# taindp98/Endoscopy-Image-Classification

Measured on AMD Instinct MI355X. Metric: unlabeled images/sec/node (FixMatch ViT-S, 224², μ=7), higher is better.
Workload: dtype bf16; 1 GPU; F1: FixMatch ViT-S/16 step, global B=64 labeled + mu*B=448 unlabeled weak/strong pairs (64 + 448 per GPU, strong scaling), 224^2, C=23, tau=0.95, lambda_u=1, Adam 1e-3, EMA 0.999; global_batch=960, seq_len=197, parallelism=dp1, hipgraph=False

## Files before the change

endoscopy-image-classification_amd/csrc/gemm.hip:

```cpp
#include <algorithm>
#include <mutex>
#include <type_traits>

#include <hip/hip_ext.h>

#include "common.h"

namespace es_gemm {

constexpr int BM = 128, BN = 128, BK = 64;

enum Epi {
  EPI_BF16 = 0,
  EPI_GELU = 1,
  EPI_F32_RESID = 2,
  EPI_DGELU = 3,
  EPI_F32 = 4,
  EPI_PATCH = 5,
  EPI_GELU_ACT = 6,
  EPI_GELU_D = 7,
  EPI_MULAUX = 8,
};

struct NTArgs {
// ... 1403 lines not shown
          const float2 rr = rv[2 * s + q / (RPS / 2)][q % (RPS / 2)][j];
          v[j] = make_float2(t.x + rr.x, t.y + rr.y);
        }
        if constexpr (s == 0)
          if (q == RPS / 2 - 1) load_resid(std::integral_constant<int, 3>{});
        const LnRow384 o = ln_row384(v, (q & 1) == 0, l.eps, gam_lds, bet_lds, lane);
        const int m = m0 + tile_row(s, q);
        const bool ok = m < p.M;
#pragma unroll
        for (int j = 0; j < 3; ++j) {
          const int c = (j * 64 + lane) * 2;
          __builtin_amdgcn_raw_buffer_store_b64(__builtin_bit_cast(u32x2, v[j]), rx,
                                                ok ? (unsigned)(m * p.ldc + c) * 4u : ES_OOB, 0, 0);
          __builtin_amdgcn_raw_buffer_store_b32(o.h[j], rh, ok ? (unsigned)(m * l.ldh + c) * 2u : ES_OOB, 0, 0);
        }
        const bool one = ok && lane == 0;
        __builtin_amdgcn_raw_buffer_store_b32(__builtin_bit_cast(unsigned, o.mean), rm,
                                              one ? (unsigned)m * 4u : ES_OOB, 0, 0);
        __builtin_amdgcn_raw_buffer_store_b32(__builtin_bit_cast(unsigned, o.rstd), rs,
                                              one ? (unsigned)m * 4u : ES_OOB, 0, 0);
      }
    };
    slab(std::integral_constant<int, 0>{});
    asm volatile("s_waitcnt lgkmcnt(0)" ::: "memory");
    __builtin_amdgcn_s_barrier();
    slab(std::integral_constant<int, 1>{});
    if (tid == 0) qslot[0] = claimed;
    asm volatile("s_waitcnt lgkmcnt(0)" ::: "memory");
    __builtin_amdgcn_s_barrier();
    cur = __builtin_amdgcn_readfirstlane(qslot[0]);
  }
  TILE_CTR_RELEASE(ctr, tid)
}
#undef TILE_CTR_RELEASE

#define NT_LAUNCH(E, BKT_, NST_, TBM_, ...)                                             \
  {                                                                                        \
    const size_t lds = std::max((size_t)NST_ * (TBM_ + BN) * BKT_ * 2, (size_t)4 * EPI_WAVE_BYTES); \
    allow_lds(gemm_nt_kernel<E, BKT_, NST_, TBM_, ##__VA_ARGS__>, lds);                   \
    hipLaunchKernelGGL(HIP_KERNEL_NAME(gemm_nt_kernel<E, BKT_, NST_, TBM_, ##__VA_ARGS__>), dim3(grid), dim3(256), lds, stream, a); \
    return ES_OK;                                                                          \
  }
#define NT_EPIS(BKT_, NST_, TBM_, ...)                                            \
  switch (epi) {                                                                  \
    case EPI_BF16: NT_LAUNCH(EPI_BF16, BKT_, NST_, TBM_, ##__VA_ARGS__)           \
    case EPI_GELU: NT_LAUNCH(EPI_GELU, BKT_, NST_, TBM_, ##__VA_ARGS__)           \
    case EPI_F32_RESID: NT_LAUNCH(EPI_F32_RESID, BKT_, NST_, TBM_, ##__VA_ARGS__) \
    case EPI_DGELU: NT_LAUNCH(EPI_DGELU, BKT_, NST_, TBM_, ##__VA_ARGS__)         \
    case EPI_F32: NT_LAUNCH(EPI_F32, BKT_, NST_, TBM_, ##__VA_ARGS__)             \
    case EPI_PATCH: NT_LAUNCH(EPI_PATCH, BKT_, NST_, TBM_, ##__VA_ARGS__)         \
    case EPI_GELU_ACT: NT_LAUNCH(EPI_GELU_ACT, BKT_, NST_, TBM_, ##__VA_ARGS__)   \
    case EPI_GELU_D: NT_LAUNCH(EPI_GELU_D, BKT_, NST_, TBM_, ##__VA_ARGS__)       \
    case EPI_MULAUX: NT_LAUNCH(EPI_MULAUX, BKT_, NST_, TBM_, ##__VA_ARGS__)       \
    default: return ES_BAD_ARG;                                                   \
  }
int launch_nt(int cfg, int epi, int grid, hipStream_t stream, const NTArgs& a) {
  if (cfg == 11 && epi == EPI_F32_RESID) NT_LAUNCH(EPI_F32_RESID, 64, 2, 64, 0)
  switch (cfg) {
    case 0: NT_EPIS(64, 2, 128)
    case 5: NT_EPIS(32, 2, 128)
    case 11: NT_EPIS(64, 2, 64)
    default: NT_EPIS(32, 3, 128)
  }
}
#undef NT_EPIS
#undef NT_LAUNCH
// ... 41 lines not shown
  if (n < CTR_SLOTS) {
    tab[n] = s;
    return n++;
  }
  return (int)(((uintptr_t)s >> 6) % CTR_SLOTS);
}
static int persistent_grid(int tiles) {
  static const int cus = [] {
    int dev = 0, n = 0;
    (void)hipGetDevice(&dev);
    return (hipDeviceGetAttribute(&n, hipDeviceAttributeMultiprocessorCount, dev) != hipSuccess || n <= 0) ? 256 : n;
  }();
  return std::max(1, std::min(cus, tiles));
}

int launch_resid_ln(hipStream_t stream, const NTArgs& a, const RLArgs& l) {
  const int grid = persistent_grid((a.M + rlg::R - 1) / rlg::R);
  allow_lds(gemm_resid_ln_kernel, (size_t)rlg::LDS);
  hipLaunchKernelGGL(gemm_resid_ln_kernel, dim3(grid), dim3(512), rlg::LDS, stream, a, l, tile_ctr_slot(stream));
  return hipGetLastError() == hipSuccess ? ES_OK : ES_HIP_ERROR;
}

int launch_nt_ln(int ring, hipStream_t stream, const NTArgs& a, const RLArgs& l) {
  const int grid = persistent_grid((a.M + nlg::TBM - 1) / nlg::TBM);
  const int slot = tile_ctr_slot(stream);
  constexpr size_t lds3 = nlg::lds<3, 32>(), lds2 = nlg::lds<2, 64>();
  if (ring == 1) {
    allow_lds(gemm_nt_ln_kernel<3, 32>, lds3);
    hipLaunchKernelGGL(HIP_KERNEL_NAME(gemm_nt_ln_kernel<3, 32>), dim3(grid), dim3(512), lds3, stream, a, l, slot);
  } else {
    allow_lds(gemm_nt_ln_kernel<2, 64>, lds2);
    hipLaunchKernelGGL(HIP_KERNEL_NAME(gemm_nt_ln_kernel<2, 64>), dim3(grid), dim3(512), lds2, stream, a, l, slot);
  }
  return hipGetLastError() == hipSuccess ? ES_OK : ES_HIP_ERROR;
}

}
using namespace es_gemm;

static int g_gemm_variant = -1;
static int g_tn_variant = -1;
static int g_small_tile = 1;

extern "C" {

int es_gemm_tn_ex(const void* A1, int ld1, const void* A2, int ld2, int M, int N1, int N2, int splits,
                  float* workspace, float* out, int accumulate, float* bias_out, int variant, hipStream_t stream);

int es_gemm_nt(int epi, const void* A, int lda, const void* B, int ldb, const float* bias, void* C,
               int ldc, void* C2, const void* aux, int ldaux, int M, int N, int K, int np,
               hipStream_t stream) {
  if (M <= 0 || N <= 0 || K <= 0 || (N % BN) || (K % BK) || (lda % 8) || (ldb % 8) || (ldc % 4))
    return ES_BAD_SHAPE;
  if (!A || !B || !C) return ES_BAD_ARG;
  if (((epi == EPI_GELU || epi == EPI_GELU_D) && !C2) ||
      ((epi == EPI_F32_RESID || epi == EPI_DGELU || epi == EPI_MULAUX || epi == EPI_PATCH) && !aux))
    return ES_BAD_ARG;
  if (epi == EPI_PATCH && np <= 0) return ES_BAD_ARG;
  if ((epi == EPI_F32_RESID || epi == EPI_PATCH) && ((ldaux % 4) || ldaux < N)) return ES_BAD_SHAPE;
  if ((epi == EPI_DGELU || epi == EPI_MULAUX) && ((ldaux % 8) || ldaux < N)) return ES_BAD_SHAPE;
  NTArgs a{(const bf16*)A, (const bf16*)B, bias, C, C2, aux, M, N, K, lda, ldb, ldc, ldaux, np};
  int variant = g_gemm_variant;
  if (variant < 0) {
    const bool gelu = epi == EPI_GELU || epi == EPI_GELU_ACT || epi == EPI_GELU_D;
    const bool plain = epi == EPI_BF16 || epi == EPI_F32 || epi == EPI_F32_RESID || epi == EPI_MULAUX;
    if (g_small_tile && N <= 384 && ((K <= 384 && epi == EPI_F32_RESID) || (M < 32768 && (plain || epi == EPI_GELU_ACT))))
// ... 56 lines not shown
      (size_t)M * (size_t)std::max(ldc, ldaux) * 4 >= (1u << 31))
    return ES_BAD_SHAPE;
  if (!A || !B || !C || !aux || !gamma || !beta || !h || !mean || !rstd) return ES_BAD_ARG;
  if ((((uintptr_t)A | (uintptr_t)aux | (uintptr_t)B | (uintptr_t)gamma | (uintptr_t)beta) & 15) ||
      (bias && ((uintptr_t)bias & 15)) || ((uintptr_t)C & 7) || ((uintptr_t)h & 3))
    return ES_BAD_ARG;
  NTArgs a{(const bf16*)A, (const bf16*)B, bias, C, nullptr, aux, M, N, K, lda, ldb, ldc, ldaux, 0};
  RLArgs l{gamma, beta, (bf16*)h, mean, rstd, ldh, eps};
  return launch_resid_ln(stream, a, l);
}

static int g_nt_ln_ring = 0;
int es_gemm_nt_ln(const void* A, int lda, const void* B, int ldb, const float* bias, float* C, int ldc,
                  const float* aux, int ldaux, const float* gamma, const float* beta, void* h, int ldh, float* mean,
                  float* rstd, int M, int N, int K, float eps, hipStream_t stream) {
  if (M <= 0 || N != nlg::D || K <= 0 || (K % 64) || (lda % 8) || (ldb % 8) || (ldc % 2) || (ldaux % 2) || (ldh % 2) ||
      lda < K || ldb < K || ldc < N || ldaux < N || ldh < N ||
      (size_t)M * (size_t)std::max(std::max(ldc, ldaux), ldh) * 4 >= (1u << 31))
    return ES_BAD_SHAPE;
  if (!A || !B || !C || !aux || !gamma || !beta || !h || !mean || !rstd) return ES_BAD_ARG;
  if ((((uintptr_t)A | (uintptr_t)B | (uintptr_t)gamma | (uintptr_t)beta) & 15) || (bias && ((uintptr_t)bias & 15)) ||
      (((uintptr_t)C | (uintptr_t)aux) & 7) || (((uintptr_t)h | (uintptr_t)mean | (uintptr_t)rstd) & 3))
    return ES_BAD_ARG;
  NTArgs a{(const bf16*)A, (const bf16*)B, bias, C, nullptr, aux, M, N, K, lda, ldb, ldc, ldaux, 0};
  RLArgs l{gamma, beta, (bf16*)h, mean, rstd, ldh, eps};
  return launch_nt_ln(g_nt_ln_ring, stream, a, l);
}
int endossl_nt_ln_ring(int v) {
  const int old = g_nt_ln_ring;
  g_nt_ln_ring = v == 1 ? 1 : 0;
  return old;
}

static bool gemm_variant_ok(int v) {
  return v == -1 || v == 0 || v == 1 || v == 2 || v == 5 || v == 6 || v == 10 || v == 11;
}
int es_set_gemm_variant(int v) {
  if (!gemm_variant_ok(v)) return ES_BAD_ARG;
  const int old = g_gemm_variant;
  g_gemm_variant = v;
  return old;
}

int es_set_gemm_small_tile(int v) {
  const int old = g_small_tile;
  g_small_tile = v;
  return old;
}

int es_set_tn_variant(int v) {
  if (v != -1 && v != 0 && v != 7) return ES_BAD_ARG;
  const int old = g_tn_variant;
  g_tn_variant = v;
  return old;
}

constexpr int TN_MIN_SPLIT_TOKENS = 512;
static bool tn_big_ok(int N1, int N2, int ld1, int ld2) {
  return N1 % TB1 == 0 && N2 % TB2 == 0 && ld1 % 8 == 0 && ld2 % 8 == 0;
}
static int tn_pick(int M, int N1, int N2, int ld1, int ld2, int v) {
  if (!(N1 % BM == 0 && N2 % BN == 0)) return 7;
  if (v == 7) return tn_big_ok(N1, N2, ld1, ld2) ? 7 : 0;
  if (v >= 0) return 0;
  return (tn_big_ok(N1, N2, ld1, ld2) && M >= 65536) ? 7 : 0;
}
// ... 259 lines not shown
```

endoscopy-image-classification_amd/endossl/_lib.py:

```python
import ctypes
import os

import torch

_HERE = os.path.dirname(os.path.abspath(__file__))
LIB_PATH = os.environ.get("ENDOSSL_LIB", os.path.join(_HERE, "lib", "libendossl_hip.so"))

V, I, L, F, Z = ctypes.c_void_p, ctypes.c_int, ctypes.c_long, ctypes.c_float, ctypes.c_size_t
U64 = ctypes.c_ulonglong

SIGNATURES = {
    "es_abi_version": (I, []),
    "es_gemm_nt": (I, [I, V, I, V, I, V, V, I, V, V, I, I, I, I, I, V]),
    "es_gemm_nt_resid_ln": (I, [V, I, V, I, V, V, I, V, I, V, V, V, I, V, V, I, I, I, F, V]),
    "es_gemm_nt_ln": (I, [V, I, V, I, V, V, I, V, I, V, V, V, I, V, V, I, I, I, F, V]),
    "es_set_gemm_variant": (I, [I]),
    "es_set_gemm_small_tile": (I, [I]),
    "es_gemm_tn_workspace": (Z, [I, I, I]),
    "es_gemm_tn": (I, [V, I, V, I, I, I, I, I, V, V, I, V, V]),
    "es_gemm_tn_ex": (I, [V, I, V, I, I, I, I, I, V, V, I, V, I, V]),
    "es_set_tn_variant": (I, [I]),
    "es_set_attn_variant": (I, [I]),
    "es_set_attn_bwd_variant": (I, [I]),
    "es_set_attn_bwd_grid": (I, [I]),
    "es_set_ln_fwd_grid": (I, [I]),
    "es_set_attn_bwd_long": (I, [I]),
    "es_splitk_reduce": (I, [V, V, I, I, I, V]),
    "es_tn_problem_size": (Z, []),
    "es_gemm_tn_grouped_prepare": (I, [V, I]),
    "es_gemm_tn_grouped": (I, [V, I, I, V]),
    "es_set_stem_kernels": (I, [I]),
    "es_gemm_tn_big_grouped_table_bytes": (Z, [I]),
    "es_gemm_tn_big_grouped_workspace": (Z, [V, I, I]),
    "es_gemm_tn_big_grouped_prepare": (I, [V, I, I, V, Z, V, V]),
    "es_gemm_tn_big_grouped": (I, [V, I, V, V]),
    "es_gemm_tn_big_grouped_timed": (I, [V, I, V, V, V, V]),
    "es_event_create": (I, [V]),
    "es_event_elapsed": (I, [V, V, V]),
    "es_event_destroy": (I, [V]),
    "es_colsum": (I, [V, I, I, I, V, I, V, I, V]),
    "es_attn_fwd": (I, [V, I, V, I, V, I, I, I, F, V]),
    "es_attn_bwd": (I, [V, I, V, I, V, V, V, I, V, I, I, I, I, F, V]),
    "es_attn_cls_fwd": (I, [V, I, V, I, V, I, I, I, F, V]),
    "es_attn_cls_bwd": (I, [V, I, V, I, V, V, I, V, I, I, I, I, F, V]),
    "es_reduce_partials": (I, [V, V, I, I, I, V]),
    "es_layernorm_fwd": (I, [V, I, V, V, V, I, V, V, I, I, F, V]),
    "es_layernorm_bwd": (I, [V, I, V, I, V, V, V, V, I, V, I, V, I, V, V, V, I, I, I, I, V]),
    "es_layernorm_bwd_b16": (I, [V, I, V, I, V, V, V, V, I, V, I, V, I, V, V, V, I, I, I, I, V]),
    "es_layernorm_bwd_grid": (I, [I, I]),
    "es_ln_param_grads_entry_size": (I, []),
    "es_ln_param_grads_multi": (I, [V, I, V]),
    "es_gelu_fwd": (I, [V, V, L, V]),
    "es_gelu_bwd": (I, [V, V, V, L, V]),
    "es_patch_im2col": (I, [V, V, I, I, I, V]),
    "es_patch_im2col_u8": (I, [V, F, F, F, F, F, F, V, I, I, I, V]),
    "es_cls_init": (I, [V, I, V, V, I, I, I, V]),
    "es_embed_bwd": (I, [V, I, V, I, V, V, I, I, I, I, V]),
    "es_cls_head_fwd": (I, [V, I, I, V, V, V, V, V, I, V, V, I, I, I, F, V]),
    "es_cls_head_bwd": (I, [V, I, V, V, V, V, V, V, V, I, I, V, V, V, V, I, I, I, V]),
    "es_cls_head_bwd_ex": (I, [V, I, V, V, V, V, V, V, V, I, I, V, V, V, V, I, I, I, I, V]),
    "es_cls_ln_fwd": (I, [V, I, I, V, V, V, I, V, V, I, I, F, V]),
    "es_cls_ln_bwd": (I, [V, I, V, V, V, V, I, I, V, V, I, I, V]),
    "es_dense_fwd": (I, [V, I, V, V, V, I, I, I, I, I, F, V, F, V]),
    "es_dense_bwd_workspace": (Z, [I, I]),
    "es_dense_bwd": (I, [V, I, V, I, I, F, V, F, V, I, V, V, I, I, V, V, I, I, I, V, V]),
    "es_bn1d_fwd": (I, [V, I, V, V, V, V, V, F, F, I, V, I, V, V, I, I, V]),
    "es_bn1d_bwd": (I, [V, I, V, V, V, V, I, V, V, I, I, V]),
    "es_dropout_keep": (I, [V, L, F, U64, U64, V]),
    "es_bn1d_sums": (I, [V, I, I, I, V, F, V, V]),
    "es_bn1d_fwd_global": (I, [V, I, V, V, V, V, F, V, V, V, F, F, V, I, V, V, I, I, V]),
    "es_bn1d_bwd_sums": (I, [V, I, V, I, I, V, V]),
    "es_bn1d_bwd_global": (I, [V, I, V, V, V, V, V, F, V, I, V, V, I, I, V]),
    "es_l2norm_fwd": (I, [V, I, V, I, V, I, I, V]),
    "es_l2norm_bwd": (I, [V, I, V, I, V, V, I, I, I, V]),
    "es_comatch_pseudo_workspace": (Z, [I, I, I]),
    "es_comatch_pseudo": (I, [V, I, I, I, V, I, I, I, V, I, I, V, V, I, F, F, F, V, V, V, V, V, V]),
    "es_comatch_pseudo_ex": (I, [V, I, I, I, V, I, I, I, I, V, I, I, V, V, I, F, F, F, V, V, V, V, V, V]),
    "es_softmax_colmean": (I, [V, I, I, I, V, V]),
    "es_comatch_bank_write": (I, [V, I, I, V, I, I, I, V, V, I, V, V, I, I, V]),
    "es_comatch_contrastive_workspace": (Z, [I]),
    "es_comatch_contrastive_fwd_bwd": (I, [V, I, V, I, V, I, I, I, F, F, F, V, V, I, V, I, V, V]),
    "es_comatch_contrastive_ex_workspace": (Z, [I, I]),
    "es_comatch_contrastive_fwd_bwd_ex": (I, [V, I, V, I, V, V, I, I, I, I, I, F, F, F, F, V, V, I, V, I, V, V]),
    "es_comatch_focal_fwd_bwd": (I, [V, I, V, V, I, I, F, F, V, V, I, V, V]),
    "es_fm_consistency_fwd_bwd": (I, [V, I, V, I, I, I, F, F, V, V, V, V, I, V, V]),
    "es_poly_ce_fwd_bwd": (I, [V, I, V, V, I, I, F, F, V, I, V, V]),
    "es_triplet_fwd_bwd": (I, [V, I, I, I, F, F, V, I, V, V]),
    "es_softmax_predict": (I, [V, I, I, I, F, V, V, V, V]),
    "es_margin_softmax_workspace": (Z, [I, I]),
# ... 194 lines not shown
```

endoscopy-image-classification_amd/endossl/vit.py:

```python
import ctypes
import functools
import math
import os

import torch
import torch.nn as nn

from . import _lib, block
from ._lib import call, ptr
from .block import (EPI_BF16, EPI_DGELU, EPI_F32, EPI_F32_RESID, EPI_GELU, EPI_GELU_ACT,
                    EPI_GELU_D, EPI_MULAUX, EPI_PATCH, Rows, _TNProblem)

LN_BWD_BLOCKS = 1024
SIDE_PRIORITY = -1
SIDE_PRIORITY_MIN_M = 65536


IMAGENET_MEAN = (0.485, 0.456, 0.406)
IMAGENET_STD = (0.229, 0.224, 0.225)


def _rup(x, m):
    return (x + m - 1) // m * m

# ... 72 lines not shown
                nn.init.uniform_(t, -bound, bound, generator=generator)
            elif name.startswith(("fc.", "head_emb.")):
                if name == "fc.3.weight":
                    t.fill_(1.0)
                elif name == "fc.3.bias":
                    t.zero_()
                elif len(shape) == 2:
                    nn.init.kaiming_uniform_(t, a=math.sqrt(5), generator=generator)
                else:
                    w = [sh for nm, sh in layout if nm == name[:-len("bias")] + "weight"][0]
                    bound = 1.0 / math.sqrt(w[1])
                    nn.init.uniform_(t, -bound, bound, generator=generator)
            elif name.startswith("head"):
                t.zero_()
            elif name.endswith("weight") and len(shape) == 2:
                nn.init.trunc_normal_(t, std=0.02, generator=generator)
            elif "norm" in name and name.endswith("weight"):
                t.fill_(1.0)
            else:
                t.zero_()


class _Acts:

    def __init__(self, cfg, n, train, device, b16=torch.bfloat16):
        D, Hd, L = cfg.dim, cfg.hidden, cfg.depth
        self.n, self.train = n, train
        self.M = n * cfg.T
        Mp = _rup(self.M, 256) + 256
        self.Mp = Mp
        Lk = L if train else 1
        f32 = torch.float32
        z = lambda *s, dt=f32: torch.zeros(*s, dtype=dt, device=device)
        self.patches = z(_rup(n * cfg.np, 256), 3 * cfg.patch * cfg.patch, dt=b16)
        self.x = z(L + 1 if train else 2, Mp, D)
        self.xmid = z(Lk, Mp, D)
        self.h1 = z(Lk, Mp, D, dt=b16)
        self.h2 = z(Lk, Mp, D, dt=b16)
        self.mean1, self.rstd1 = z(Lk, Mp), z(Lk, Mp)
        self.mean2, self.rstd2 = z(Lk, Mp), z(Lk, Mp)
        self.qkv = z(Lk, Mp, 3 * D, dt=b16)
        self.o = z(Lk, Mp, D, dt=b16)
        self.lse = z(Lk, n * cfg.heads * cfg.T)
        self.pre = z(Lk if train else 0, Mp, Hd, dt=b16)
        self.act = z(Lk, Mp, Hd, dt=b16)
        Mc = _rup(n, 256)
        self.c_o, self.c_lse = z(Mc, D, dt=b16), z(n * cfg.heads)
        self.c_h1 = z(Mc, D, dt=b16)
        self.c_xmid, self.c_h2 = z(Mc, D), z(Mc, D, dt=b16)
        self.c_mean2, self.c_rstd2 = z(Mc), z(Mc)
        self.c_pre = z(Mc, Hd, dt=b16) if train else None
        self.c_act, self.c_xout = z(Mc, Hd, dt=b16), z(Mc, D)
        self.xhat = z(n, D)
        self.rstd_cls = z(n)
        self.logits = z(n, cfg.num_classes)
        self.fts = z(n, D) if cfg.head == "emb" else None


class _Grads:

    def __init__(self, cfg, n, device, b16=torch.bfloat16):
        D, Hd = cfg.dim, cfg.hidden
        Mp = _rup(n * cfg.T, 256) + 256
        f32 = torch.float32
        z = lambda *s, dt=f32: torch.zeros(*s, dtype=dt, device=device)
        self.n = n
        self.dx, self.dxb = z(Mp, D), z(Mp, D, dt=b16)
        self.dxm, self.dxmb = z(Mp, D), z(Mp, D, dt=b16)
        self.dh = z(Mp, D, dt=b16) if Engine.DH_BF16 else z(Mp, D)
        self.dpre = z(Mp, Hd, dt=b16)
        self.dqkv = z(Mp, 3 * D, dt=b16)
        self.do = z(Mp, D, dt=b16)
        self.dpatch = z(_rup(n * cfg.np, 256), D, dt=b16)
        self.dyn = z(n, D)
        self.delta = z(n * cfg.heads * cfg.T)
        Mc = _rup(n, 256)
        self.c_dx, self.c_dxb = z(Mc, D), z(Mc, D, dt=b16)
        self.c_dpre, self.c_dxmb, self.c_do = z(Mc, Hd, dt=b16), z(Mc, D, dt=b16), z(Mc, D, dt=b16)
        self.c_dh = z(Mc, D, dt=b16) if Engine.DH_BF16 else z(Mc, D)
        self.dxm_cls = z(Mp, D)


class _WgradSchedule:

    def __init__(self, sets, M, depth, grouped, *, layer_wgrad, defer_ln, bf16, capture, group_layers, min_m, main,
                 side, wgrad, wgrad_layer, launch_grouped, ln_flush, grad_ready=None, block_range=None,
                 on_stream=block.on_stream):
        self.mode = "grouped" if grouped else "layer" if layer_wgrad and bf16 and M >= min_m else "each"
        self.defer = [] if defer_ln and grad_ready is None and not capture and self.mode != "each" else None
# ... 52 lines not shown
            self._launch_grouped(self.problems, 0)
        if self.defer:
            self._ln_flush(self.defer)
        if self.side is not None:
            self.main.wait_stream(self.side)


class Engine:

    TN_TARGET_BLOCKS = 768
    TN_SHARE = 0.5
    TN_SHARE_MIN_M = 16384
    TN_MAX_SPLITS = 128
    GROUP_WGRAD = "auto"
    GROUP_WGRAD_MAX_M = 16384
    GROUP_LAYERS = 6
    DEFER_LN_GRADS = True
    LN_MULTI_MAX = 32
    LAYER_WGRAD = True
    LAYER_TN_SHARE = 0.375
    _OV = os.environ.get("ENDOSSL_OVERLAP", "1")
    OVERLAP_FWD = _OV in ("1", "fwd")
    OVERLAP = _OV in ("1", "bwd")
    DH_BF16 = True
    GELU_D = True
    PRUNE_LAST = True
    PRUNE_Q = True
    RESID_LN = os.environ.get("ENDOSSL_RESID_LN", "1") == "1"
    RESID_LN_MIN_M = 40000
    FC2_LN = os.environ.get("ENDOSSL_FC2_LN", "1") == "1"
    FC2_LN_MIN_M = 50000
    FC2_LN_TRAIN = True
    FC2_LN_WEAK = True

    PARITY_NAMES = {n: n + "_f32" for n in (
        "es_gemm_nt", "es_gemm_tn", "es_attn_fwd", "es_attn_bwd", "es_attn_cls_fwd", "es_attn_cls_bwd",
        "es_layernorm_fwd", "es_layernorm_bwd", "es_patch_im2col", "es_patch_im2col_u8", "es_embed_bwd",
        "es_pack_weights")}
    PARITY_NAMES.update({"es_layernorm_bwd_b16": "es_layernorm_bwd_f32", "es_cast_f32_bf16": "es_copy_f32"})

    def __init__(self, cfg, device, precision="bf16"):
        if precision not in ("bf16", "fp32"):
            raise ValueError(f"precision must be 'bf16' (production) or 'fp32' (parity mode), got {precision!r}")
        self.cfg, self.device = cfg, device
        self.precision = precision
        self.op_dtype = torch.bfloat16 if precision == "bf16" else torch.float32
        self.layout, self.offs, self.numel = param_layout(cfg)
        self.shapes = dict(self.layout)
        self._acts = {}
        self._grads = {}
        self._ws = None
        self._ws_ln = None
        self._ws_lnp = None
        self._lnp_next = 0
        self._side = None
        self._ncu_cache = None
        self._gtab = {}
        self._grad_b = None
        self.overlap = self.OVERLAP
        self.overlap_fwd = self.OVERLAP_FWD
        self._packed_version = -1
        D, Hd = cfg.dim, cfg.hidden
        b16 = self.op_dtype
        mats = [("patch_embed.proj.weight", D, 3 * cfg.patch * cfg.patch, False)]
        for i in range(cfg.depth):
            b = f"blocks.{i}."
# ... 58 lines not shown
        if self._ws is None:
            cfg = self.cfg
            D, Hd = cfg.dim, cfg.hidden
            n_tn = max(a * b for a, b in ((3 * D, D), (D, D), (Hd, D), (D, Hd), (D, 3 * cfg.patch * cfg.patch)))
            self._ws = torch.empty(self.TN_MAX_SPLITS * n_tn + 2 * 1024 * max(Hd, 3 * D), dtype=torch.float32,
                                   device=self.device)
        return self._ws

    def ln_workspace(self):
        if self._ws_ln is None:
            self._ws_ln = torch.empty(2 * LN_BWD_BLOCKS * self.cfg.dim, dtype=torch.float32, device=self.device)
        return self._ws_ln

    def _ncu(self):
        if self._ncu_cache is None:
            self._ncu_cache = torch.cuda.get_device_properties(self.device).multi_processor_count
        return self._ncu_cache

    def side_stream(self, tokens=0):
        prio = SIDE_PRIORITY if tokens >= SIDE_PRIORITY_MIN_M else 0
        if self._side is None:
            self._side = {}
        if prio not in self._side:
            self._side[prio] = torch.cuda.Stream(device=self.device, priority=prio)
        return self._side[prio]

    def forward(self, flat, images_list, train):
        cfg = self.cfg
        s = _lib.stream()
        n = sum(int(t.shape[0]) for t in images_list)
        A = self.acts(n, train)
        D, T, H = cfg.dim, cfg.T, cfg.heads
        K0 = 3 * cfg.patch * cfg.patch
        row = 0
        for t in images_list:
            if t.shape[1:] != (3, cfg.img_size, cfg.img_size) or t.dtype not in (torch.float32, torch.uint8):
                raise ValueError(f"expected fp32 (normalised) or uint8 (raw) [n,3,{cfg.img_size},{cfg.img_size}] "
                                 f"images, got {tuple(t.shape)} {t.dtype}")
            t = t.contiguous()
            if t.dtype == torch.uint8:
                self._call("es_patch_im2col_u8", ptr(t), *IMAGENET_MEAN, *IMAGENET_STD, ptr(A.patches[row * cfg.np:]),
                     int(t.shape[0]), cfg.img_size, cfg.patch, s)
            else:
                self._call("es_patch_im2col", ptr(t), ptr(A.patches[row * cfg.np:]), int(t.shape[0]), cfg.img_size,
                     cfg.patch, s)
            row += int(t.shape[0])
        x0 = A.x[0]
        pos = self.view(flat, "pos_embed")
        block.gemm_nt(self._call, EPI_PATCH, A.patches, self.wb["patch_embed.proj.weight"],
                      self.view(flat, "patch_embed.proj.bias"), x0, n * cfg.np, D, K0, aux=pos, ldaux=D, npatch=cfg.np)
        self._call("es_cls_init", ptr(x0), D, ptr(self.view(flat, "cls_token")), ptr(pos), n, T, D, s)
        M = A.M
        prune = self._prune()
        ch = self._chain(flat)
        fused = self.RESID_LN and D == 384 and self.precision == "bf16" and M >= self.RESID_LN_MIN_M
        fc2_ln = (self.FC2_LN and (self.FC2_LN_TRAIN if train else self.FC2_LN_WEAK) and D == 384
                  and self.precision == "bf16" and M >= self.FC2_LN_MIN_M)
        ln_done = False
        for i in range(cfg.depth):
            b = f"blocks.{i}."
            li = i if train else 0
            xin = A.x[i] if train else A.x[i & 1]
            xout = A.x[i + 1] if train else A.x[(i + 1) & 1]
            R = Rows(n, T, H, x=xin, h1=A.h1[li], mean1=A.mean1[li], rstd1=A.rstd1[li], qkv=A.qkv[li], o=A.o[li],
                     lse=A.lse[li], xmid=A.xmid[li], h2=A.h2[li], mean2=A.mean2[li], rstd2=A.rstd2[li],
                     pre=A.pre[li] if train else None, act=A.act[li], out=xout)
            if prune and i == cfg.depth - 1:
                Rc = self._cls_rows(A, n, xin)
                ch.attn_fwd(b, R, cls=Rc, split_q=self.PRUNE_Q, ln_done=ln_done)
                ch.mlp_fwd(b, Rc, train)
                if self.capture is not None:
                    self.capture("fwd_cls", train, i, xin[:M], A.c_xout[:n])
                break
            ch.attn_fwd(b, R, ln_done=ln_done)
            next_ln = None
            if fc2_ln and i + 1 < cfg.depth:
                nb, ni = f"blocks.{i + 1}.", i + 1 if train else 0
                next_ln = (self.view(flat, nb + "norm1.weight"), self.view(flat, nb + "norm1.bias"), A.h1[ni],
                           A.mean1[ni], A.rstd1[ni])
            ch.mlp_fwd(b, R, train, fused=fused, label="fc1_fwd" if train else "fc1_fwd_weak", next_ln=next_ln)
            ln_done = next_ln is not None
            if self.capture is not None:
                self.capture("fwd", train, i, xin[:M], xout[:M])
        xl = A.x[cfg.depth] if train else A.x[cfg.depth & 1]
        Tl = T
        if prune:
            xl, Tl = A.c_xout, 1
        if cfg.head == "emb":
            self._call("es_cls_ln_fwd", ptr(xl), D, Tl, ptr(self.view(flat, "norm.weight")),
                 ptr(self.view(flat, "norm.bias")), ptr(A.fts), D, ptr(A.xhat), ptr(A.rstd_cls), n, D, cfg.eps, s)
            return A.fts
# ... 346 lines not shown
```

include/endossl.h:

```cpp
#ifndef ENDOSSL_H
#define ENDOSSL_H
#include <stddef.h>
#include <stdint.h>
#include <hip/hip_runtime_api.h>

#ifdef __cplusplus
extern "C" {
#endif

int es_abi_version(void);

int es_gemm_nt(int epi, const void* A, int lda, const void* B, int ldb, const float* bias, void* C, int ldc,
               void* C2, const void* aux, int ldaux, int M, int N, int K, int np, hipStream_t stream);
int es_gemm_nt_resid_ln(const void* A, int lda, const void* B, int ldb, const float* bias, float* C, int ldc,
                        const float* aux, int ldaux, const float* gamma, const float* beta, void* h, int ldh,
                        float* mean, float* rstd, int M, int N, int K, float eps, hipStream_t stream);
int es_gemm_nt_ln(const void* A, int lda, const void* B, int ldb, const float* bias, float* C, int ldc,
                  const float* aux, int ldaux, const float* gamma, const float* beta, void* h, int ldh, float* mean,
                  float* rstd, int M, int N, int K, float eps, hipStream_t stream);
int es_set_gemm_variant(int variant);
int es_set_gemm_small_tile(int v);
int es_set_tn_variant(int variant);
size_t es_gemm_tn_workspace(int N1, int N2, int splits);
int es_gemm_tn(const void* A1, int ld1, const void* A2, int ld2, int M, int N1, int N2, int splits,
// ... 54 lines not shown
int es_ln_param_grads_entry_size(void);
int es_ln_param_grads_multi(const void* table, int n, hipStream_t stream);

int es_gelu_fwd(const void* x, void* y, long n, hipStream_t stream);
int es_gelu_bwd(const void* x, const void* dy, void* dx, long n, hipStream_t stream);

size_t es_aug_entry_size(void);
size_t es_aug_strong_workspace(int n, int S);
size_t es_aug_fixmatch_workspace(int n, int S, int is_crop, int max_w, int max_h);
int es_aug_fixmatch_u8(const uint8_t* frames, size_t frames_bytes, const void* entries, const int32_t* coeffs,
                       size_t coeff_count, int n, int S, int is_crop, int max_h, uint8_t* weak, uint8_t* strong,
                       void* workspace, size_t workspace_bytes, hipStream_t stream);
int es_aug_strong_u8(const uint8_t* weak, const void* entries, int n, int S, uint8_t* strong, void* workspace,
                     size_t workspace_bytes, hipStream_t stream);

size_t es_aug_comatch_entry_size(void);
size_t es_aug_labeled_entry_size(void);
size_t es_aug_comatch_workspace(int n, int S, int is_crop, int max_w, int max_h);
size_t es_aug_labeled_workspace(int n, int S, int is_crop, int max_w, int max_h);
int es_aug_comatch_u8(const uint8_t* frames, size_t frames_bytes, const void* entries, const int32_t* coeffs,
                      size_t coeff_count, int n, int S, int is_crop, int max_h, uint8_t* weak, uint8_t* strong0,
                      uint8_t* strong1, void* workspace, size_t workspace_bytes, hipStream_t stream);
int es_aug_labeled_u8(const uint8_t* frames, size_t frames_bytes, const void* entries, const int32_t* coeffs,
                      size_t coeff_count, int n, int S, int is_crop, int max_h, uint8_t* out, void* workspace,
                      size_t workspace_bytes, hipStream_t stream);
int es_aug_jitter_u8(const uint8_t* x, const void* plans, int n, int S, uint8_t* out, hipStream_t stream);


int es_patch_im2col(const float* img, void* patches, int n, int S, int P, hipStream_t stream);

int es_patch_im2col_u8(const void* img, float mean0, float mean1, float mean2, float std0, float std1, float std2,
                       void* patches, int n, int S, int P, hipStream_t stream);
int es_cls_init(float* x, int ldx, const float* cls, const float* pos, int n, int T, int D, hipStream_t stream);
int es_embed_bwd(const float* dx, int lddx, void* dpatch, int ldp, float* dpos, float* dcls, int n, int T, int D,
                 int accumulate, hipStream_t stream);
int es_cls_head_fwd(const float* x, int ldx, int T, const float* gamma, const float* beta, const float* W,
                    const float* b, float* logits, int ldl, float* xhat, float* rstd, int n, int D, int C, float eps,
                    hipStream_t stream);
int es_cls_head_bwd(const float* dl, int lddl, const float* W, const float* gamma, const float* beta,
                    const float* xhat, const float* rstd, float* dyn, float* dx, int lddx, int T, float* dW, float* db,
                    float* dgamma, float* dbeta, int n, int D, int C, hipStream_t stream);
int es_cls_head_bwd_ex(const float* dl, int lddl, const float* W, const float* gamma, const float* beta,
                       const float* xhat, const float* rstd, float* dyn, float* dx, int lddx, int T, float* dW,
                       float* db, float* dgamma, float* dbeta, int n, int D, int C, int accumulate, hipStream_t stream);

int es_cls_ln_fwd(const float* x, int ldx, int T, const float* gamma, const float* beta, float* fts, int ldf,
                  float* xhat, float* rstd, int n, int D, float eps, hipStream_t stream);
int es_cls_ln_bwd(const float* dfts, int lddf, const float* gamma, const float* xhat, const float* rstd, float* dx,
                  int lddx, int T, float* dgamma, float* dbeta, int n, int D, hipStream_t stream);

int es_dense_fwd(const float* X, int ldx, const float* W, const float* b, float* Y, int ldy, int n, int K, int N,
                 int act, float slope, const void* keep, float keep_scale, hipStream_t stream);
size_t es_dense_bwd_workspace(int n, int N);
int es_dense_bwd(const float* dY, int lddy, const float* Yact, int ldya, int act, float slope, const void* keep,
                 float keep_scale, const float* X, int ldx, const float* W, float* dX, int lddx, int accumulate_dx,
                 float* dW, float* db, int n, int K, int N, float* workspace, hipStream_t stream);
int es_bn1d_fwd(const float* U, int ldu, const float* gamma, const float* beta, float* running_mean, float* running_var,
                void* num_batches_tracked, float momentum, float eps, int train, float* Y, int ldy, float* xhat,
                float* rstd, int n, int F, hipStream_t stream);
int es_bn1d_bwd(const float* dY, int lddy, const float* xhat, const float* rstd, const float* gamma, float* dU,
                int lddu, float* dgamma, float* dbeta, int n, int F, hipStream_t stream);
int es_bn1d_sums(const float* U, int ldu, int n, int F, const float* S1, float N, float* out, hipStream_t stream);
int es_bn1d_fwd_global(const float* U, int ldu, const float* gamma, const float* beta, const float* S1,
                       const float* S2, float N, float* running_mean, float* running_var, void* num_batches_tracked,
                       float momentum, float eps, float* Y, int ldy, float* xhat, float* rstd, int n, int F,
                       hipStream_t stream);
// ... 267 lines not shown
```

Measured before the change: 15380 unlabeled images/s.

## Fuse uint8 im2col, patch-embed GEMM, pos add and first LayerNorm into one kernel

Adds a persistent patch-embedding kernel that reads raw uint8 images directly, normalises them through an LDS lookup table into the GEMM A tile, adds bias and positional embedding, and computes block 0's norm1 LayerNorm in the epilogue. A companion kernel writes the CLS row plus its LayerNorm, and the patch buffer is allocated lazily and only written when training needs it for the backward pass. This removes the separate im2col pass, one activation round trip and a standalone LayerNorm launch, at the cost of a more complex kernel with per-thread image address computation and gathered A loads instead of async global-to-LDS copies.

```diff
diff --git a/endoscopy-image-classification_amd/csrc/gemm.hip b/endoscopy-image-classification_amd/csrc/gemm.hip
--- a/endoscopy-image-classification_amd/csrc/gemm.hip
+++ b/endoscopy-image-classification_amd/csrc/gemm.hip
@@ -1459,6 +1459,266 @@
   }
   TILE_CTR_RELEASE(ctr, tid)
 }
+
+struct PEArgs {
+  const uint8_t* img[4];
+  int pstart[4];
+  int S, G, np;
+  float mean[3], std[3];
+  bf16* patches;
+};
+namespace peg {
+constexpr int BKT = 64, NST = 2, KD = 768;
+constexpr int BODY = nlg::body<NST, BKT>();
+constexpr int LDS = BODY + 16 + nlg::D * 4 * 3 + 3 * 256 * 2;
+}
+
+__global__ __launch_bounds__(512, 1) void patch_embed_ln_kernel(NTArgs p, RLArgs l, PEArgs e, int slot) {
+  using namespace nlg;
+  constexpr int BKT = peg::BKT;
+  extern __shared__ __attribute__((aligned(16))) char smem[];
+  constexpr int ROWB = BKT * 2, RPI = 1024 / ROWB, CPR = ROWB / 16, RPW = 8 * RPI;
+  constexpr int IB = D / RPW;
+  constexpr int TA = TBM * ROWB, STAGE = (TBM + D) * ROWB;
+  int* const qslot = (int*)(smem + peg::BODY);
+  float* const bias_lds = (float*)(smem + peg::BODY + 16);
+  float* const gam_lds = bias_lds + D;
+  float* const bet_lds = gam_lds + D;
+  unsigned short* const tab = (unsigned short*)(bet_lds + D);
+  const int tid = threadIdx.x, lane = tid & 63;
+  const int w = __builtin_amdgcn_readfirstlane(tid >> 6);
+  const int wm = w / WN, wn = w % WN;
+  const int g = lane >> 4, r = lane & 15;
+  int* const ctr = g_tile_ctr + slot * CTR_INTS;
+  const int nt = (p.M + TBM - 1) / TBM;
+  if (tid == 0) qslot[0] = __hip_atomic_fetch_add(ctr, 1, __ATOMIC_RELAXED, __HIP_MEMORY_SCOPE_AGENT);
+  if (tid < D / 4) {
+    *(f32x4*)(bias_lds + 4 * tid) = p.bias ? *(const f32x4*)(p.bias + 4 * tid) : f32x4{0.f, 0.f, 0.f, 0.f};
+    *(f32x4*)(gam_lds + 4 * tid) = *(const f32x4*)(l.gamma + 4 * tid);
+    *(f32x4*)(bet_lds + 4 * tid) = *(const f32x4*)(l.beta + 4 * tid);
+  }
+  for (int i = tid; i < 3 * 256; i += 512) {
+    const int c = i >> 8;
+    const float mu = c == 0 ? e.mean[0] : (c == 1 ? e.mean[1] : e.mean[2]);
+    const float sd = c == 0 ? e.std[0] : (c == 1 ? e.std[1] : e.std[2]);
+    const bf16 v = (bf16)(((float)(i & 255) / 255.0f - mu) / sd);
+    tab[i] = __builtin_bit_cast(unsigned short, v);
+  }
+  __syncthreads();
+  int cur = __builtin_amdgcn_readfirstlane(qslot[0]);
+
+  const bf16* gb[IB];
+#pragma unroll
+  for (int j = 0; j < IB; ++j) {
+    const int row = (j * 8 + w) * RPI + lane / CPR;
+    gb[j] = p.B + (size_t)row * p.ldb + swzk<BKT>(row, lane % CPR) * 8;
+  }
+  const int pr = tid >> 2, kyi = tid & 3;
+  const unsigned aoff0 = pr * ROWB + (swzk<BKT>(pr, 2 * kyi) << 4), aoff1 = pr * ROWB + (swzk<BKT>(pr, 2 * kyi + 1) << 4);
+  const unsigned T = (unsigned)e.np + 1u, rows = (unsigned)(p.M / e.np) * T;
+  const __amdgpu_buffer_rsrc_t rx = buf_rsrc(p.C, rows * p.ldc * 4u);
+  const __amdgpu_buffer_rsrc_t rh = buf_rsrc(l.h, rows * l.ldh * 2u);
+  const __amdgpu_buffer_rsrc_t rm = buf_rsrc(l.mean, rows * 4u);
+  const __amdgpu_buffer_rsrc_t rs = buf_rsrc(l.rstd, rows * 4u);
+  const __amdgpu_buffer_rsrc_t rp = buf_rsrc(e.patches ? (void*)e.patches : p.C, e.patches ? (unsigned)p.M * peg::KD * 2u : 0u);
+  const float* const pos = (const float*)p.aux;
+  constexpr int nk = peg::KD / BKT;
+  const size_t plane = (size_t)e.S * e.S;
+
+  while (cur < nt) {
+    const int m0 = cur * TBM, last = p.M - 1;
+    auto tile_row = [&](int s, int q) {
+      const int lr = w * RPS + q;
+      return (lr >> 5) * 64 + s * 32 + (lr & 31);
+    };
+    float2 rv[4][RPS / 2][3];
+    auto load_pos = [&](auto gc) {
+      constexpr int gi = decltype(gc)::value;
+#pragma unroll
+      for (int q = 0; q < RPS / 2; ++q) {
+        const int mm = min(m0 + tile_row(gi >> 1, (gi & 1) * (RPS / 2) + q), last);
+        const float* xr = pos + (size_t)(1 + mm % e.np) * p.ldaux;
+#pragma unroll
+        for (int j = 0; j < 3; ++j) rv[gi][q][j] = *(const float2*)(xr + (j * 64 + lane) * 2);
+      }
+    };
+
+    const int am = min(m0 + pr, last);
+    const int ti = (am >= e.pstart[1]) + (am >= e.pstart[2]) + (am >= e.pstart[3]);
+    const uint8_t* const ib = ti == 0 ? e.img[0] : (ti == 1 ? e.img[1] : (ti == 2 ? e.img[2] : e.img[3]));
+    const int lm = am - (ti == 0 ? e.pstart[0] : (ti == 1 ? e.pstart[1] : (ti == 2 ? e.pstart[2] : e.pstart[3])));
+    const int im = lm / e.np, pi = lm - im * e.np, py = pi / e.G, px = pi - py * e.G;
+    const uint8_t* const asrc = ib + (size_t)im * 3 * plane + (size_t)(py * 16 + kyi) * e.S + px * 16;
+    const unsigned poff = (e.patches && m0 + pr <= last) ? (unsigned)((m0 + pr) * peg::KD + kyi * 16) * 2u : ES_OOB;
+    auto a_load = [&](int kt) { return *(const u32x4*)(asrc + (size_t)(kt >> 2) * plane + (size_t)((kt & 3) * 4) * e.S); };
+    auto a_put = [&](int buf, int kt, u32x4 raw) {
+      const unsigned short* tb = tab + (kt >> 2) * 256;
+      u32x4 o[2];
+#pragma unroll
+      for (int j = 0; j < 8; ++j) {
+        const unsigned v = raw[j >> 1] >> (16 * (j & 1));
+        o[j >> 2][j & 3] = (unsigned)tb[v & 255u] | ((unsigned)tb[(v >> 8) & 255u] << 16);
+      }
+      char* S_ = smem + buf * STAGE;
+      *(u32x4*)(S_ + aoff0) = o[0];
+      *(u32x4*)(S_ + aoff1) = o[1];
+      const unsigned po = poff == ES_OOB ? ES_OOB : poff + kt * BKT * 2;
+      __builtin_amdgcn_raw_buffer_store_b128(o[0], rp, po, 0, 0);
+      __builtin_amdgcn_raw_buffer_store_b128(o[1], rp, po == ES_OOB ? ES_OOB : po + 16, 0, 0);
+    };
+#define PE_ISSUE_B(BUF, K0)                                                                              \
+  {                                                                                                      \
+    char* S_ = smem + (BUF) * STAGE;                                                                     \
+    _Pragma("unroll") for (int j = 0; j < IB; ++j) glds16(gb[j] + (K0), S_ + TA + (j * 8 + w) * 1024);   \
+  }
+    f32x4 acc[MF][NF];
+#pragma unroll
+    for (int i = 0; i < MF; ++i)
+#pragma unroll
+      for (int j = 0; j < NF; ++j) acc[i][j] = f32x4{0.f, 0.f, 0.f, 0.f};
+    u32x4 raw = a_load(0), raw2;
+    PE_ISSUE_B(0, 0)
+    a_put(0, 0, raw);
+    asm volatile("" ::: "memory");
+    raw = a_load(1);
+    raw2 = a_load(2);
+    int buf = 0;
+    for (int kt = 0; kt < nk; ++kt) {
+      if (kt + 2 < nk) asm volatile("s_waitcnt vmcnt(1) lgkmcnt(0)" ::: "memory");
+      else asm volatile("s_waitcnt vmcnt(0) lgkmcnt(0)" ::: "memory");
+      __builtin_amdgcn_s_barrier();
+      if (kt + 1 < nk) {
+        const int nb = buf ^ 1;
+        PE_ISSUE_B(nb, (kt + 1) * BKT)
+        a_put(nb, kt + 1, raw);
+        raw = raw2;
+        asm volatile("" ::: "memory");
+        if (kt + 3 < nk) raw2 = a_load(kt + 3);
+      }
+      const char* As = smem + buf * STAGE;
+      const char* Bs = As + TA;
+#pragma unroll
+      for (int kk = 0; kk < BKT / 32; ++kk) {
+        bf16x8 af[MF], bfr[NF];
+#pragma unroll
+        for (int j = 0; j < NF; ++j) {
+          const int rb = wn * NF * 16 + j * 16 + r;
+          bfr[j] = *(const bf16x8*)(Bs + rb * ROWB + swzk<BKT>(rb, kk * 4 + g) * 16);
+        }
+#pragma unroll
+        for (int i = 0; i < MF; ++i) {
+          const int ra = wm * MF * 16 + i * 16 + r;
+          af[i] = *(const bf16x8*)(As + ra * ROWB + swzk<BKT>(ra, kk * 4 + g) * 16);
+        }
+        __builtin_amdgcn_s_setprio(1);
+#pragma unroll
+        for (int i = 0; i < MF; ++i)
+#pragma unroll
+          for (int j = 0; j < NF; ++j) acc[i][j] = mfma16(bfr[j], af[i], acc[i][j]);
+        __builtin_amdgcn_s_setprio(0);
+      }
+      buf ^= 1;
+    }
+#undef PE_ISSUE_B
+    asm volatile("s_waitcnt lgkmcnt(0)" ::: "memory");
+    __builtin_amdgcn_s_barrier();
+    int claimed = 0;
+    if (tid == 0) claimed = __hip_atomic_fetch_add(ctr, 1, __ATOMIC_RELAXED, __HIP_MEMORY_SCOPE_AGENT);
+    load_pos(std::integral_constant<int, 0>{});
+    load_pos(std::integral_constant<int, 1>{});
+
+    auto slab = [&](auto sc) {
+      constexpr int s = decltype(sc)::value;
+#pragma unroll
+      for (int i = 0; i < 2; ++i)
+#pragma unroll
+        for (int j = 0; j < NF; ++j) {
+          const int lr = wm * 32 + i * 16 + r, c = wn * NF * 4 + 4 * j + g;
+          *(f32x4*)(smem + lr * ROWX + ((c ^ r) << 4)) =
+              acc[2 * s + i][j] + *(const f32x4*)(bias_lds + wn * NF * 16 + 16 * j + 4 * g);
+        }
+      if constexpr (s == 0) load_pos(std::integral_constant<int, 2>{});
+      asm volatile("s_waitcnt lgkmcnt(0)" ::: "memory");
+      __builtin_amdgcn_s_barrier();
+#pragma unroll
+      for (int q = 0; q < RPS; ++q) {
+        const int lr = w * RPS + q;
+        float2 v[3];
+#pragma unroll
+        for (int j = 0; j < 3; ++j) {
+          const int cc = (j * 64 + lane) >> 1;
+          const float2 t = *(const float2*)(smem + lr * ROWX + ((cc ^ (lr & 15)) << 4) + (lane & 1) * 8);
+          const float2 rr = rv[2 * s + q / (RPS / 2)][q % (RPS / 2)][j];
+          v[j] = make_float2(t.x + rr.x, t.y + rr.y);
+        }
+        if constexpr (s == 0)
+          if (q == RPS / 2 - 1) load_pos(std::integral_constant<int, 3>{});
+        const int mp = m0 + tile_row(s, q);
+        const bool ok = mp < p.M;
+        const int mi = min(mp, last) / e.np;
+        const int m = mi * (int)T + 1 + (min(mp, last) - mi * e.np);
+        const LnRow384 o = ln_row384(v, (m & 1) == 0, l.eps, gam_lds, bet_lds, lane);
+#pragma unroll
+        for (int j = 0; j < 3; ++j) {
+          const int c = (j * 64 + lane) * 2;
+          __builtin_amdgcn_raw_buffer_store_b64(__builtin_bit_cast(u32x2, v[j]), rx,
+                                                ok ? (unsigned)(m * p.ldc + c) * 4u : ES_OOB, 0, 0);
+          __builtin_amdgcn_raw_buffer_store_b32(o.h[j], rh, ok ? (unsigned)(m * l.ldh + c) * 2u : ES_OOB, 0, 0);
+        }
+        const bool one = ok && lane == 0;
+        __builtin_amdgcn_raw_buffer_store_b32(__builtin_bit_cast(unsigned, o.mean), rm,
+                                              one ? (unsigned)m * 4u : ES_OOB, 0, 0);
+        __builtin_amdgcn_raw_buffer_store_b32(__builtin_bit_cast(unsigned, o.rstd), rs,
+                                              one ? (unsigned)m * 4u : ES_OOB, 0, 0);
+      }
+    };
+    slab(std::integral_constant<int, 0>{});
+    asm volatile("s_waitcnt lgkmcnt(0)" ::: "memory");
+    __builtin_amdgcn_s_barrier();
+    slab(std::integral_constant<int, 1>{});
+    if (tid == 0) qslot[0] = claimed;
+    asm volatile("s_waitcnt lgkmcnt(0)" ::: "memory");
+    __builtin_amdgcn_s_barrier();
+    cur = __builtin_amdgcn_readfirstlane(qslot[0]);
+  }
+  TILE_CTR_RELEASE(ctr, tid)
+}
+
+__global__ __launch_bounds__(256) void cls_init_ln_kernel(float* __restrict__ x, int ldx, const float* __restrict__ cls,
+                                                          const float* __restrict__ pos, const float* __restrict__ gamma,
+                                                          const float* __restrict__ beta, bf16* __restrict__ h, int ldh,
+                                                          float* __restrict__ mean, float* __restrict__ rstd, int n, int T,
+                                                          float eps) {
+  __shared__ float gb_lds[2 * nlg::D];
+  for (int i = threadIdx.x; i < nlg::D; i += 256) {
+    gb_lds[i] = gamma[i];
+    gb_lds[nlg::D + i] = beta[i];
+  }
+  __syncthreads();
+  const int lane = threadIdx.x & 63;
+  float2 v[3];
+#pragma unroll
+  for (int j = 0; j < 3; ++j) {
+    const int c = (j * 64 + lane) * 2;
+    v[j] = make_float2(cls[c] + pos[c], cls[c + 1] + pos[c + 1]);
+  }
+  const LnRow384 oe = ln_row384(v, true, eps, gb_lds, gb_lds + nlg::D, lane);
+  const LnRow384 oo = ln_row384(v, false, eps, gb_lds, gb_lds + nlg::D, lane);
+  for (int im = blockIdx.x * 4 + (threadIdx.x >> 6); im < n; im += gridDim.x * 4) {
+    const size_t m = (size_t)im * T;
+    const bool even = (m & 1) == 0;
+#pragma unroll
+    for (int j = 0; j < 3; ++j) {
+      const int c = (j * 64 + lane) * 2;
+      *(float2*)(x + m * ldx + c) = v[j];
+      *(unsigned*)(h + m * ldh + c) = even ? oe.h[j] : oo.h[j];
+    }
+    if (lane == 0) {
+      mean[m] = even ? oe.mean : oo.mean;
+      rstd[m] = even ? oe.rstd : oo.rstd;
+    }
+  }
+}
 #undef TILE_CTR_RELEASE
 
 #define NT_LAUNCH(E, BKT_, NST_, TBM_, ...)                                             \
@@ -1566,6 +1826,13 @@
     allow_lds(gemm_nt_ln_kernel<2, 64>, lds2);
     hipLaunchKernelGGL(HIP_KERNEL_NAME(gemm_nt_ln_kernel<2, 64>), dim3(grid), dim3(512), lds2, stream, a, l, slot);
   }
+  return hipGetLastError() == hipSuccess ? ES_OK : ES_HIP_ERROR;
+}
+
+int launch_patch_embed_ln(hipStream_t stream, const NTArgs& a, const RLArgs& l, const PEArgs& e) {
+  const int grid = persistent_grid((a.M + nlg::TBM - 1) / nlg::TBM);
+  allow_lds(patch_embed_ln_kernel, (size_t)peg::LDS);
+  hipLaunchKernelGGL(patch_embed_ln_kernel, dim3(grid), dim3(512), peg::LDS, stream, a, l, e, tile_ctr_slot(stream));
   return hipGetLastError() == hipSuccess ? ES_OK : ES_HIP_ERROR;
 }
 
@@ -1688,6 +1955,53 @@
   return old;
 }
 
+int es_patch_embed_ln_u8(const void* const* imgs, const int* counts, int nsrc, int S, float mean0, float mean1,
+                         float mean2, float std0, float std1, float std2, const void* W, int ldw, const float* bias,
+                         const float* pos, int ldpos, const float* gamma, const float* beta, float eps, float* x,
+                         int ldx, void* h, int ldh, float* mean, float* rstd, void* patches, hipStream_t stream) {
+  if (nsrc < 1 || nsrc > 4 || !imgs || !counts) return ES_BAD_ARG;
+  if (S <= 0 || (S % 16) || (ldw % 8) || ldw < peg::KD || (ldx % 2) || ldx < nlg::D || (ldh % 2) || ldh < nlg::D ||
+      (ldpos % 2) || ldpos < nlg::D)
+    return ES_BAD_SHAPE;
+  if (!W || !pos || !gamma || !beta || !x || !h || !mean || !rstd) return ES_BAD_ARG;
+  PEArgs e{};
+  e.S = S;
+  e.G = S / 16;
+  e.np = e.G * e.G;
+  size_t n = 0;
+  for (int i = 0; i < nsrc; ++i) {
+    if (!imgs[i] || ((uintptr_t)imgs[i] & 15) || counts[i] <= 0) return ES_BAD_ARG;
+    e.img[i] = (const uint8_t*)imgs[i];
+    e.pstart[i] = (int)(n * e.np);
+    n += (size_t)counts[i];
+    if (n * (size_t)(e.np + 1) * (size_t)std::max(ldx, ldh) * 4 >= (1u << 31)) return ES_BAD_SHAPE;
+  }
+  const int M = (int)(n * e.np);
+  for (int i = nsrc; i < 4; ++i) {
+    e.img[i] = e.img[0];
+    e.pstart[i] = M;
+  }
+  if ((((uintptr_t)W | (uintptr_t)gamma | (uintptr_t)beta | (uintptr_t)patches) & 15) || (bias && ((uintptr_t)bias & 15)) ||
+      (((uintptr_t)x | (uintptr_t)pos) & 7) || (((uintptr_t)h | (uintptr_t)mean | (uintptr_t)rstd) & 3))
+    return ES_BAD_ARG;
+  e.mean[0] = mean0; e.mean[1] = mean1; e.mean[2] = mean2;
+  e.std[0] = std0; e.std[1] = std1; e.std[2] = std2;
+  e.patches = (bf16*)patches;
+  NTArgs a{nullptr, (const bf16*)W, bias, x, nullptr, pos, M, nlg::D, peg::KD, 0, ldw, ldx, ldpos, e.np};
+  RLArgs l{gamma, beta, (bf16*)h, mean, rstd, ldh, eps};
+  return launch_patch_embed_ln(stream, a, l, e);
+}
+
+int es_cls_init_ln(float* x, int ldx, const float* cls, const float* pos, const float* gamma, const float* beta, void* h,
+                   int ldh, float* mean, float* rstd, int n, int T, int D, float eps, hipStream_t stream) {
+  if (n <= 0 || T <= 0 || D != nlg::D || (ldx % 2) || ldx < D || (ldh % 2) || ldh < D) return ES_BAD_SHAPE;
+  if (!x || !cls || !pos || !gamma || !beta || !h || !mean || !rstd) return ES_BAD_ARG;
+  if (((uintptr_t)x & 7) || ((uintptr_t)h & 3)) return ES_BAD_ARG;
+  hipLaunchKernelGGL(cls_init_ln_kernel, dim3(std::min((n + 3) / 4, 256)), dim3(256), 0, stream, x, ldx, cls, pos, gamma,
+                     beta, (bf16*)h, ldh, mean, rstd, n, T, eps);
+  return hipGetLastError() == hipSuccess ? ES_OK : ES_HIP_ERROR;
+}
+
 static bool gemm_variant_ok(int v) {
   return v == -1 || v == 0 || v == 1 || v == 2 || v == 5 || v == 6 || v == 10 || v == 11;
 }
diff --git a/endoscopy-image-classification_amd/endossl/_lib.py b/endoscopy-image-classification_amd/endossl/_lib.py
--- a/endoscopy-image-classification_amd/endossl/_lib.py
+++ b/endoscopy-image-classification_amd/endossl/_lib.py
@@ -55,6 +55,8 @@
     "es_patch_im2col": (I, [V, V, I, I, I, V]),
     "es_patch_im2col_u8": (I, [V, F, F, F, F, F, F, V, I, I, I, V]),
     "es_cls_init": (I, [V, I, V, V, I, I, I, V]),
+    "es_patch_embed_ln_u8": (I, [V, V, I, I, F, F, F, F, F, F, V, I, V, V, I, V, V, F, V, I, V, I, V, V, V, V]),
+    "es_cls_init_ln": (I, [V, I, V, V, V, V, V, I, V, V, I, I, I, F, V]),
     "es_embed_bwd": (I, [V, I, V, I, V, V, I, I, I, I, V]),
     "es_cls_head_fwd": (I, [V, I, I, V, V, V, V, V, I, V, V, I, I, I, F, V]),
     "es_cls_head_bwd": (I, [V, I, V, V, V, V, V, V, V, I, I, V, V, V, V, I, I, I, V]),
diff --git a/endoscopy-image-classification_amd/endossl/vit.py b/endoscopy-image-classification_amd/endossl/vit.py
--- a/endoscopy-image-classification_amd/endossl/vit.py
+++ b/endoscopy-image-classification_amd/endossl/vit.py
@@ -128,7 +128,8 @@
         Lk = L if train else 1
         f32 = torch.float32
         z = lambda *s, dt=f32: torch.zeros(*s, dtype=dt, device=device)
-        self.patches = z(_rup(n * cfg.np, 256), 3 * cfg.patch * cfg.patch, dt=b16)
+        self._patches = None
+        self._patches_new = lambda: z(_rup(n * cfg.np, 256), 3 * cfg.patch * cfg.patch, dt=b16)
         self.x = z(L + 1 if train else 2, Mp, D)
         self.xmid = z(Lk, Mp, D)
         self.h1 = z(Lk, Mp, D, dt=b16)
@@ -151,6 +152,12 @@
         self.rstd_cls = z(n)
         self.logits = z(n, cfg.num_classes)
         self.fts = z(n, D) if cfg.head == "emb" else None
+
+    @property
+    def patches(self):
+        if self._patches is None:
+            self._patches = self._patches_new()
+        return self._patches
 
 
 class _Grads:
@@ -269,6 +276,8 @@
     FC2_LN_MIN_M = 50000
     FC2_LN_TRAIN = True
     FC2_LN_WEAK = True
+    PATCH_LN = os.environ.get("ENDOSSL_PATCH_LN", "1") == "1"
+    PATCH_LN_MIN_M = 20000
 
     PARITY_NAMES = {n: n + "_f32" for n in (
         "es_gemm_nt", "es_gemm_tn", "es_attn_fwd", "es_attn_bwd", "es_attn_cls_fwd", "es_attn_cls_bwd",
@@ -393,8 +402,11 @@
         A = self.acts(n, train)
         D, T, H = cfg.dim, cfg.T, cfg.heads
         K0 = 3 * cfg.patch * cfg.patch
+        patch_ln = (self.PATCH_LN and D == 384 and cfg.patch == 16 and self.precision == "bf16" and cfg.depth > 0
+                    and A.M >= self.PATCH_LN_MIN_M and 1 <= len(images_list) <= 4
+                    and all(t.dtype == torch.uint8 for t in images_list))
         row = 0
-        for t in images_list:
+        for t in () if patch_ln else images_list:
             if t.shape[1:] != (3, cfg.img_size, cfg.img_size) or t.dtype not in (torch.float32, torch.uint8):
                 raise ValueError(f"expected fp32 (normalised) or uint8 (raw) [n,3,{cfg.img_size},{cfg.img_size}] "
                                  f"images, got {tuple(t.shape)} {t.dtype}")
@@ -408,16 +420,33 @@
             row += int(t.shape[0])
         x0 = A.x[0]
         pos = self.view(flat, "pos_embed")
-        block.gemm_nt(self._call, EPI_PATCH, A.patches, self.wb["patch_embed.proj.weight"],
-                      self.view(flat, "patch_embed.proj.bias"), x0, n * cfg.np, D, K0, aux=pos, ldaux=D, npatch=cfg.np)
-        self._call("es_cls_init", ptr(x0), D, ptr(self.view(flat, "cls_token")), ptr(pos), n, T, D, s)
+        if patch_ln:
+            imgs = []
+            for t in images_list:
+                if t.shape[1:] != (3, cfg.img_size, cfg.img_size):
+                    raise ValueError(f"expected uint8 [n,3,{cfg.img_size},{cfg.img_size}] images, got {tuple(t.shape)}")
+                imgs.append(t.contiguous())
+            tab = (ctypes.c_void_p * len(imgs))(*[ptr(t) for t in imgs])
+            cnt = (ctypes.c_int * len(imgs))(*[int(t.shape[0]) for t in imgs])
+            g1, b1 = self.view(flat, "blocks.0.norm1.weight"), self.view(flat, "blocks.0.norm1.bias")
+            self._call("es_cls_init_ln", ptr(x0), D, ptr(self.view(flat, "cls_token")), ptr(pos), ptr(g1), ptr(b1),
+                       ptr(A.h1[0]), D, ptr(A.mean1[0]), ptr(A.rstd1[0]), n, T, D, cfg.eps, s)
+            self._call("es_patch_embed_ln_u8", tab, cnt, len(imgs), cfg.img_size, *IMAGENET_MEAN, *IMAGENET_STD,
+                       ptr(self.wb["patch_embed.proj.weight"]), K0, ptr(self.view(flat, "patch_embed.proj.bias")),
+                       ptr(pos), D, ptr(g1), ptr(b1), cfg.eps, ptr(x0), D, ptr(A.h1[0]), D, ptr(A.mean1[0]),
+                       ptr(A.rstd1[0]), ptr(A.patches) if train else None, s)
+        else:
+            block.gemm_nt(self._call, EPI_PATCH, A.patches, self.wb["patch_embed.proj.weight"],
+                          self.view(flat, "patch_embed.proj.bias"), x0, n * cfg.np, D, K0, aux=pos, ldaux=D,
+                          npatch=cfg.np)
+            self._call("es_cls_init", ptr(x0), D, ptr(self.view(flat, "cls_token")), ptr(pos), n, T, D, s)
         M = A.M
         prune = self._prune()
         ch = self._chain(flat)
         fused = self.RESID_LN and D == 384 and self.precision == "bf16" and M >= self.RESID_LN_MIN_M
         fc2_ln = (self.FC2_LN and (self.FC2_LN_TRAIN if train else self.FC2_LN_WEAK) and D == 384
                   and self.precision == "bf16" and M >= self.FC2_LN_MIN_M)
-        ln_done = False
+        ln_done = patch_ln
         for i in range(cfg.depth):
             b = f"blocks.{i}."
             li = i if train else 0
diff --git a/include/endossl.h b/include/endossl.h
--- a/include/endossl.h
+++ b/include/endossl.h
@@ -110,6 +110,13 @@
 int es_patch_im2col_u8(const void* img, float mean0, float mean1, float mean2, float std0, float std1, float std2,
                        void* patches, int n, int S, int P, hipStream_t stream);
 int es_cls_init(float* x, int ldx, const float* cls, const float* pos, int n, int T, int D, hipStream_t stream);
+
+int es_patch_embed_ln_u8(const void* const* imgs, const int* counts, int nsrc, int S, float mean0, float mean1,
+                         float mean2, float std0, float std1, float std2, const void* W, int ldw, const float* bias,
+                         const float* pos, int ldpos, const float* gamma, const float* beta, float eps, float* x,
+                         int ldx, void* h, int ldh, float* mean, float* rstd, void* patches, hipStream_t stream);
+int es_cls_init_ln(float* x, int ldx, const float* cls, const float* pos, const float* gamma, const float* beta, void* h,
+                   int ldh, float* mean, float* rstd, int n, int T, int D, float eps, hipStream_t stream);
 int es_embed_bwd(const float* dx, int lddx, void* dpatch, int ldp, float* dpos, float* dcls, int n, int T, int D,
                  int accumulate, hipStream_t stream);
 int es_cls_head_fwd(const float* x, int ldx, int T, const float* gamma, const float* beta, const float* W,
```

New measurement: 15390 unlabeled images/s (median of 3 runs). No clear change (+0.0%).
